# pyxploiter/HandMvNet

Hardware: AMD Instinct MI355X
Metric: samples/sec (BxV frames) eval_fps.py, 8-view 256x256; 21-kpt L2 vs reference (higher is better)
Workload: dtype f32; 1 GPU; BASELINE configs[2]: B=32/GPU x V=8 x 256x256, resnet50_paper backbone, d=524, cross_attn x5, GCN decoder; global_batch=32, views=8, frame=256, parallelism=sample-shard x1

## Files before the change

handmvnet_amd/csrc/conv_stream.hip:

```cpp
#include <cstdio>
#include <cstdlib>
#include <type_traits>
#include <utility>

#include "kernels.h"

namespace hmv {

typedef float sf32x16 __attribute__((ext_vector_type(16)));
typedef float sf32x4 __attribute__((ext_vector_type(4)));
typedef _Float16 sf16x8 __attribute__((ext_vector_type(8)));

#define HMV_SGLDS16(gptr, lptr)                                                                             \
    __builtin_amdgcn_global_load_lds((const __attribute__((address_space(1))) void *)(gptr),                \
                                     (__attribute__((address_space(3))) void *)(lptr), 16, 0, 0)

template <int N>
__device__ __forceinline__ void wait_vm() {
    static_assert(N >= 0 && N < 64, "vmcnt is a 6-bit field");
    asm volatile("s_waitcnt vmcnt(%0)" ::"n"(N) : "memory");
}
template <typename F, int... I>
__device__ __forceinline__ void static_for_impl(F &&f, std::integer_sequence<int, I...>) {
    (f(std::integral_constant<int, I>{}), ...);
}
template <int N, typename F>
__device__ __forceinline__ void static_for(F &&f) {
    static_for_impl(static_cast<F &&>(f), std::make_integer_sequence<int, N>{});
}

constexpr int sched_r(int RB, int RS, int j) { return RS ? RS : (j == 0 ? RB : 0); }
constexpr int sched_ops(int NP, int PA, int RB, int RS, int OS, int slot) { return slot < NP ? PA + sched_r(RB, RS, slot) : OS; }
constexpr int sched_after_piece(int NP, int D, int PA, int RB, int RS, int OS, int j) {
    const int T0 = 8, g = T0 * NP + j - D, tq = g / NP, jq = g - tq * NP;
    int n = sched_r(RB, RS, jq);
    for (int s = tq * (NP + 1) + jq + 1; s < T0 * (NP + 1) + j; ++s) n += sched_ops(NP, PA, RB, RS, OS, s % (NP + 1));
    return n;
}
constexpr int sched_after_residual(int NP, int PA, int RB, int RS, int OS) {
    const int T0 = 8, last = RS ? NP - 1 : 0;
    int n = 0;
    for (int s = (T0 - 1) * (NP + 1) + last + 1; s < T0 * (NP + 1) + NP; ++s) n += sched_ops(NP, PA, RB, RS, OS, s % (NP + 1));
    return n;
}
static_assert(sched_after_piece(4, 3, 1, 8, 0, 8, 0) == 10 && sched_after_piece(4, 3, 1, 8, 0, 8, 1) == 18 && sched_after_piece(4, 3, 1, 8, 0, 8, 2) == 18 &&
              sched_after_piece(4, 3, 1, 8, 0, 8, 3) == 10 && sched_after_residual(4, 1, 8, 0, 8) == 23, "the step-0 schedule of four pieces, counted by hand");
static_assert(sched_after_piece(4, 3, 1, 8, 2, 8, 0) == 2 + 3 + 3 + 8 && sched_after_residual(4, 1, 8, 2, 8) == 8 + 4 * 3, "the spread K = 256 schedule");

template <int TM, int TN, int MW, int NW, int NP, int NSLOT, bool HAS_RES, bool SPREAD = false, bool DUAL = false, int N2 = 0>
__global__ __launch_bounds__(64 * MW *NW, (MW * NW) / 4) void conv_stream_f16(const ConvParams p) {
    constexpr int NWV = MW * NW, NT = 64 * NWV;
    constexpr int BM = 32 * TM * MW, BN = 32 * TN * NW;
    constexpr int D = NSLOT - 1;
    constexpr int PA = BM * 8 / NT;
    constexpr int NB2 = N2 / 32;
    constexpr int TM2 = N2 ? (BM / 32) * NB2 / NWV : 0;
    constexpr int K2Q = BN / 16;
    static_assert(N2 == 0 || (N2 % 32 == 0 && TN == 2 && TM2 >= 1 && NWV % NB2 == 0 && (BM / 32) == (NWV / NB2) * TM2),
                  "chain: a wave's 64 output channels are one pixel piece of the second reduction; whole blocks per wave");
    constexpr int RB = HAS_RES ? TM * TN * 2 : 0, OS = TM * TN * 2 + 2 * TM2;
    constexpr int RS = (SPREAD && HAS_RES) ? RB / NP : 0;
    static_assert(!SPREAD || RB % NP == 0, "spread schedule: whole residual DMAs per step");
    constexpr int ZW = TM * TN * 2 * 1024;
    constexpr int NFAKE = (D + NP - 1) / NP;
    static_assert(NT == 512 && BM % 64 == 0 && PA >= 1, "eight waves; whole DMA passes per piece");
    static_assert((NSLOT & (NSLOT - 1)) == 0 && NSLOT >= 2, "a power of two");
    extern __shared__ __attribute__((aligned(16))) char ssm[];
    _Float16 *sA = reinterpret_cast<_Float16 *>(ssm);
    char *zones = ssm + NSLOT * BM * 128;

    const int tid = threadIdx.x, lane = tid & 63;
    const int wave = __builtin_amdgcn_readfirstlane(tid >> 6);
    const int l31 = lane & 31, kh = lane >> 5;
    const int mw = wave / NW, nw = wave - mw * NW;
    const int zi = N2 ? nw * MW + mw : wave;
    static_assert(N2 == 0 || !HAS_RES || ZW == TM * 32 * 128, "chain: a landing zone is the wave's region of the tile image");

    const int nsl = p.ntiles;
    const int loc = (int)blockIdx.x >> 3, per_xcd = 32 / nsl;
    const int slice = loc % nsl, stream = ((int)blockIdx.x & 7) * per_xcd + loc / nsl, nstreams = 8 * per_xcd;
    const int ntl = p.mtiles > stream ? (p.mtiles - stream + nstreams - 1) / nstreams : 0;
    if (ntl == 0) return;
    const int n0 = slice * BN + nw * TN * 32;

    const _Float16 *zero16 = reinterpret_cast<const _Float16 *>(p.zero);
    _Float16 *trash = reinterpret_cast<_Float16 *>(const_cast<float *>(p.zero) + 64 + 4 * lane);
    const _Float16 *Ain = reinterpret_cast<const _Float16 *>(p.in);
    const _Float16 *Rin = reinterpret_cast<const _Float16 *>(p.res);
    _Float16 *Out = reinterpret_cast<_Float16 *>(p.out);

    const int wl31 = (l31 & 0x13) | ((l31 & 4) << 1) | ((l31 & 8) >> 1);
    sf16x8 wreg[TN][NP * 4];
    {
        const _Float16 *wb = reinterpret_cast<const _Float16 *>(p.wgt) + (size_t)(n0 + wl31) * p.ldw + 8 * kh;
#pragma unroll
        for (int b = 0; b < TN; ++b)
#pragma unroll
            for (int Q = 0; Q < NP * 4; ++Q) wreg[b][Q] = *reinterpret_cast<const sf16x8 *>(wb + (size_t)(32 * b) * p.ldw + 16 * Q);
    }
    const int ob2 = N2 ? wave % (N2 ? NB2 : 1) : 0, pg2 = N2 ? wave / (N2 ? NB2 : 1) : 0;
    sf16x8 w2reg[N2 ? K2Q : 1];
    if constexpr (N2 > 0) {
        const _Float16 *wb2 = reinterpret_cast<const _Float16 *>(p.nx_wgt) + (size_t)(32 * ob2 + wl31) * p.nx_ldw + 8 * kh;
#pragma unroll
        for (int Q = 0; Q < K2Q; ++Q) w2reg[Q] = *reinterpret_cast<const sf16x8 *>(wb2 + 16 * Q);
    }
    asm volatile("s_waitcnt vmcnt(0)" ::: "memory");

    const int arow = tid >> 3, kqs = (tid & 7) ^ ((tid >> 4) & 7);
    const int fsw = (l31 >> 1) & 7;

    size_t off2[DUAL ? PA : 1] = {};
    auto issue_A = [&](int G) {
        const int tt = G >= 0 ? G / NP : -1, jj = G >= 0 ? G - tt * NP : 0, slot = G & (NSLOT - 1);
        const int mt = stream + tt * nstreams;
#pragma unroll
        for (int i = 0; i < PA; ++i) {
            const int m = mt * BM + i * 64 + arow;
            const bool ok = tt >= 0 && tt < ntl && m < p.M;
            const _Float16 *src = zero16;
            if constexpr (DUAL) {
                if (jj * 64 == p.ksplit) {
                    const int hw = p.Ho * p.Wo, n = m / hw, rem = m - n * hw, ho = rem / p.Wo, wo = rem - ho * p.Wo;
                    off2[i] = ((size_t)(n * p.H2 + ho * p.stride2) * p.W2 + wo * p.stride2) * p.lda2 + 8 * kqs;
                }
                if (ok && jj * 64 >= p.ksplit) {
                    src = reinterpret_cast<const _Float16 *>(p.in2) + off2[i] + (jj * 64 - p.ksplit);
                } else if (ok) {
                    src = Ain + (size_t)m * p.lda + jj * 64 + 8 * kqs;
                }
            } else if (ok) {
                src = Ain + (size_t)m * p.lda + jj * 64 + 8 * kqs;
            }
            asm volatile("" : "+v"(src));
            HMV_SGLDS16(src, sA + ((slot * BM + i * 64 + wave * 8) * 64));
        }
    };
    auto issue_R = [&](int tt, auto first_c, auto count_c) {
        if constexpr (HAS_RES) {
            constexpr int first = decltype(first_c)::value, count = decltype(count_c)::value;
            const int mt = stream + tt * nstreams;
            char *z = zones + ((tt & 1) * NWV + zi) * ZW;
#pragma unroll
            for (int idx = first; idx < first + count; ++idx) {
                const int a = idx / (2 * TN), b = (idx / 2) % TN, j = idx & 1;
                const int m = mt * BM + (mw * TM + a) * 32 + l31;
                const bool ok = tt >= 0 && tt < ntl && m < p.M;
                const _Float16 *src = ok ? Rin + (size_t)m * p.ldr + n0 + 32 * b + 16 * j + 8 * kh : zero16;
                asm volatile("" : "+v"(src));
                HMV_SGLDS16(src, z + idx * 1024);
            }
        }
    };
    using I0 = std::integral_constant<int, 0>;
    using IRB = std::integral_constant<int, RB>;
    using IRS = std::integral_constant<int, RS>;

#pragma unroll
    for (int ft = -NFAKE; ft < 0; ++ft) {
        static_for<NP>([&](auto jc) {
            constexpr int j = decltype(jc)::value;
            issue_A(ft * NP + j + D);
            if constexpr (RS > 0) issue_R(ft + 1, std::integral_constant<int, j * RS>{}, IRS{});
            else if constexpr (j == 0) issue_R(ft + 1, I0{}, IRB{});
        });
#pragma unroll
        for (int i = 0; i < OS; ++i)
            asm volatile("global_store_dwordx4 %0, %1, off\n\ts_nop 1" ::"v"(trash), "v"(sf32x4{0.f, 0.f, 0.f, 0.f}) : "memory");
    }

    const float lo = (p.act == ACT_RELU) ? 0.f : -INFINITY;
    const __attribute__((address_space(4))) float *bp0 =
        (const __attribute__((address_space(4))) float *)(p.bias + __builtin_amdgcn_readfirstlane(n0));
    sf32x16 acc[TM][TN];

    for (int tt = 0; tt < ntl; ++tt) {
        int bz;
        asm volatile("s_mov_b32 %0, 0" : "=s"(bz));
        const __attribute__((address_space(4))) float *bp = bp0 + bz;
#pragma unroll
        for (int b = 0; b < TN; ++b)
#pragma unroll
            for (int e = 0; e < 16; ++e) {
                const int c = 32 * b + 16 * (e >> 3) + (e & 7);
                const float v0 = bp[c], v1 = bp[c + 8];
                const float v = kh ? v1 : v0;
#pragma unroll
                for (int a = 0; a < TM; ++a) acc[a][b][e] = v;
            }
        static_for<NP>([&](auto jc) {
            constexpr int j = decltype(jc)::value;
            wait_vm<sched_after_piece(NP, D, PA, RB, RS, OS, j)>();
            asm volatile("s_waitcnt lgkmcnt(0)\n\ts_barrier" ::: "memory");
            issue_A(tt * NP + j + D);
            if constexpr (RS > 0) issue_R(tt + 1, std::integral_constant<int, j * RS>{}, IRS{});
            else if constexpr (j == 0) issue_R(tt + 1, I0{}, IRB{});
            const _Float16 *pa = sA + ((((tt * NP + j) & (NSLOT - 1)) * BM + mw * TM * 32 + l31) * 64);
#pragma unroll
            for (int q = 0; q < 4; ++q) {
                sf16x8 px[TM];
#pragma unroll
                for (int a = 0; a < TM; ++a) px[a] = *reinterpret_cast<const sf16x8 *>(pa + a * 32 * 64 + (((2 * q + kh) ^ fsw) * 8));
#pragma unroll
                for (int a = 0; a < TM; ++a)
#pragma unroll
                    for (int b = 0; b < TN; ++b)
                        acc[a][b] = __builtin_amdgcn_mfma_f32_32x32x16_f16(wreg[b][4 * j + q], px[a], acc[a][b], 0, 0, 0);
            }
        });
        if constexpr (HAS_RES) wait_vm<sched_after_residual(NP, PA, RB, RS, OS)>();
        const int mt = stream + tt * nstreams;
        const char *z = zones + ((tt & 1) * NWV + zi) * ZW + lane * 16;
        if constexpr (N2 > 0) {
            char *yt = HAS_RES ? zones + (tt & 1) * NWV * ZW : zones;
            sf16x8 rr[TM][TN][2], hv[TM][TN][2];
            if constexpr (HAS_RES) {
#pragma unroll
                for (int a = 0; a < TM; ++a)
#pragma unroll
                    for (int b = 0; b < TN; ++b)
#pragma unroll
                        for (int j = 0; j < 2; ++j) rr[a][b][j] = *reinterpret_cast<const sf16x8 *>(z + ((a * TN + b) * 2 + j) * 1024);
            }
#pragma unroll
            for (int a = 0; a < TM; ++a) {
                const int m = mt * BM + (mw * TM + a) * 32 + l31;
                _Float16 *orow = Out + (size_t)m * p.ldc + n0 + 8 * kh;
#pragma unroll
                for (int b = 0; b < TN; ++b)
#pragma unroll
                    for (int j = 0; j < 2; ++j) {
                        sf16x8 r = {0, 0, 0, 0, 0, 0, 0, 0};
                        if constexpr (HAS_RES) r = rr[a][b][j];
#pragma unroll
                        for (int u = 0; u < 8; ++u) hv[a][b][j][u] = (_Float16)fmaxf(acc[a][b][8 * j + u] * p.acc_scale + (float)r[u], lo);
                        _Float16 *dst = m < p.M ? orow + 32 * b + 16 * j : trash;
                        asm volatile("global_store_dwordx4 %0, %1, off\n\ts_nop 1" ::"v"(dst), "v"(hv[a][b][j]) : "memory");
                        if constexpr (!HAS_RES) {
                            const unsigned ya = (unsigned)(size_t)(__attribute__((address_space(3))) char *)yt +
                                                (unsigned)((nw * BM + (mw * TM + a) * 32 + l31) * 128 + (((4 * b + 2 * j + kh) ^ fsw) * 16));
                            asm volatile("ds_write_b128 %0, %1" ::"v"(ya), "v"(hv[a][b][j]) : "memory");
                        }
                    }
            }
            if constexpr (HAS_RES) {
#pragma unroll
            for (int a = 0; a < TM; ++a)
#pragma unroll
                for (int b = 0; b < TN; ++b)
#pragma unroll
                    for (int j = 0; j < 2; ++j) {
                        const unsigned ya = (unsigned)(size_t)(__attribute__((address_space(3))) char *)yt +
                                            (unsigned)((nw * BM + (mw * TM + a) * 32 + l31) * 128 + (((4 * b + 2 * j + kh) ^ fsw) * 16));
                        asm volatile("ds_write_b128 %0, %1" ::"v"(ya), "v"(hv[a][b][j]) : "memory");
                    }
            }
            asm volatile("s_waitcnt lgkmcnt(0)\n\ts_barrier" ::: "memory");
            const __attribute__((address_space(4))) float *bq =
                (const __attribute__((address_space(4))) float *)(p.nx_bias + __builtin_amdgcn_readfirstlane(32 * ob2)) + bz;
            sf32x16 acc2[TM2];
#pragma unroll
            for (int e = 0; e < 16; ++e) {
                const int c = 16 * (e >> 3) + (e & 7);
                const float v0 = bq[c], v1 = bq[c + 8];
                const float v = kh ? v1 : v0;
#pragma unroll
                for (int a = 0; a < TM2; ++a) acc2[a][e] = v;
            }
            const unsigned yr = (unsigned)(size_t)(__attribute__((address_space(3))) char *)yt + (unsigned)((pg2 * TM2 * 32 + l31) * 128);
            constexpr int G = 4 / TM2, NG = K2Q / G;
            static_assert(K2Q % G == 0 && G * TM2 == 4, "four fragment reads per group");
            sf16x8 px[2][G][TM2];
#define HMV_CHAIN_READ_GROUP(g)                                                                                                     \
    _Pragma("unroll") for (int i = 0; i < G; ++i) _Pragma("unroll") for (int a = 0; a < TM2; ++a) {                                \
        const int Q = (g) * G + i;                                                                                                  \
        const unsigned ad = yr + (unsigned)(((Q >> 2) * BM + a * 32) * 128) + (unsigned)((((2 * (Q & 3) + kh) ^ fsw)) * 16);        \
        asm volatile("ds_read_b128 %0, %1" : "=v"(px[(g) & 1][i][a]) : "v"(ad) : "memory");                                         \
    }
            HMV_CHAIN_READ_GROUP(0)
#pragma unroll
            for (int g = 0; g < NG; ++g) {
                sf16x8(&pg)[G][TM2] = px[g & 1];
                if (g + 1 < NG) {
                    HMV_CHAIN_READ_GROUP(g + 1)
                    if constexpr (TM2 == 1) asm volatile("s_waitcnt lgkmcnt(4)" : "+v"(pg[0][0]), "+v"(pg[1][0]), "+v"(pg[2][0]), "+v"(pg[3][0]) :: "memory");
                    else asm volatile("s_waitcnt lgkmcnt(4)" : "+v"(pg[0][0]), "+v"(pg[0][1]), "+v"(pg[1][0]), "+v"(pg[1][1]) :: "memory");
                } else {
                    if constexpr (TM2 == 1) asm volatile("s_waitcnt lgkmcnt(0)" : "+v"(pg[0][0]), "+v"(pg[1][0]), "+v"(pg[2][0]), "+v"(pg[3][0]) :: "memory");
                    else asm volatile("s_waitcnt lgkmcnt(0)" : "+v"(pg[0][0]), "+v"(pg[0][1]), "+v"(pg[1][0]), "+v"(pg[1][1]) :: "memory");
                }
#pragma unroll
                for (int i = 0; i < G; ++i)
#pragma unroll
                    for (int a = 0; a < TM2; ++a) acc2[a] = __builtin_amdgcn_mfma_f32_32x32x16_f16(w2reg[g * G + i], pg[i][a], acc2[a], 0, 0, 0);
            }
#undef HMV_CHAIN_READ_GROUP
            const float lo2 = (p.nx_act == ACT_RELU) ? 0.f : -INFINITY;
            _Float16 *Out2 = reinterpret_cast<_Float16 *>(p.nx_out);
#pragma unroll
            for (int a = 0; a < TM2; ++a) {
                const int m = mt * BM + (pg2 * TM2 + a) * 32 + l31;
                _Float16 *orow = Out2 + (size_t)m * p.nx_ldc + 32 * ob2 + 8 * kh;
#pragma unroll
                for (int j = 0; j < 2; ++j) {
                    const sf16x8 r = {0, 0, 0, 0, 0, 0, 0, 0};
                    sf16x8 h2;
#pragma unroll
                    for (int u = 0; u < 8; ++u) h2[u] = (_Float16)fmaxf(acc2[a][8 * j + u] * p.acc_scale + (float)r[u], lo2);
                    _Float16 *dst = m < p.M ? orow + 16 * j : trash;
                    asm volatile("global_store_dwordx4 %0, %1, off\n\ts_nop 1" ::"v"(dst), "v"(h2) : "memory");
                }
            }
        } else {
#pragma unroll
        for (int a = 0; a < TM; ++a) {
            const int m = mt * BM + (mw * TM + a) * 32 + l31;
            _Float16 *orow = Out + (size_t)m * p.ldc + n0 + 8 * kh;
#pragma unroll
            for (int b = 0; b < TN; ++b)
#pragma unroll
                for (int j = 0; j < 2; ++j) {
                    sf16x8 r = {0, 0, 0, 0, 0, 0, 0, 0};
                    if constexpr (HAS_RES) r = *reinterpret_cast<const sf16x8 *>(z + ((a * TN + b) * 2 + j) * 1024);
                    sf16x8 hv;
#pragma unroll
                    for (int u = 0; u < 8; ++u) hv[u] = (_Float16)fmaxf(acc[a][b][8 * j + u] * p.acc_scale + (float)r[u], lo);
                    _Float16 *dst = m < p.M ? orow + 32 * b + 16 * j : trash;
                    asm volatile("global_store_dwordx4 %0, %1, off\n\ts_nop 1" ::"v"(dst), "v"(hv) : "memory");
                }
        }
        }
    }
    asm volatile("s_waitcnt vmcnt(0) lgkmcnt(0)" ::: "memory");
}

template <int TM, int TN, int MW, int NW, int NP, int NSLOT, bool HAS_RES, bool DUAL = false, bool HALF = false>
__global__ __launch_bounds__(64 * MW *NW, 2) void conv_stream_f32(const ConvParams p) {
    constexpr int NWV = MW * NW, NT = 64 * NWV;
    constexpr int BM = 32 * TM * MW, BN = 32 * TN * NW;
    constexpr int D = NSLOT - 1;
    constexpr int PA = BM * 8 / NT;
    constexpr int RB = HAS_RES ? TM * TN * 4 : 0, OS = TM * TN * 4, RS = 0;
    constexpr int ZW = TM * TN * 4 * 1024;
    constexpr int NFAKE = (D + NP - 1) / NP;
    constexpr int RPP = NT / 8;
    static_assert((NT == 512 || (HALF && NT == 256)) && BM % RPP == 0 && PA >= 1 && (!HALF || (HAS_RES && !DUAL)), "whole DMA passes per piece");
    static_assert((NSLOT & (NSLOT - 1)) == 0 && NSLOT >= 2, "a power of two");
    extern __shared__ __attribute__((aligned(16))) char ssm[];
    float *sA = reinterpret_cast<float *>(ssm);
    char *zones = ssm + NSLOT * BM * 128;

    const int tid = threadIdx.x, lane = tid & 63;
    const int wave = __builtin_amdgcn_readfirstlane(tid >> 6);
    const int l31 = lane & 31, kh = lane >> 5;
    const int mw = wave / NW, nw = wave - mw * NW;
    const int nsl = p.ntiles;
    const int loc = (int)blockIdx.x >> 3, per_xcd = ((int)gridDim.x >> 3) / nsl;
    const int slice = loc % nsl, stream = ((int)blockIdx.x & 7) * per_xcd + loc / nsl, nstreams = 8 * per_xcd;
    const int ntl = p.mtiles > stream ? (p.mtiles - stream + nstreams - 1) / nstreams : 0;
    if (ntl == 0) return;
    const int n0 = slice * BN + nw * TN * 32;

    const float *zero32 = p.zero;
    float *trash = const_cast<float *>(p.zero) + 64 + 4 * lane;
    const float *Ain = reinterpret_cast<const float *>(p.in);
    const float *Rin = reinterpret_cast<const float *>(p.res);
    float *Out = reinterpret_cast<float *>(p.out);

    sf32x4 wreg[TN][NP * 4], bias[TN][4];
    {
        const float *wb = reinterpret_cast<const float *>(p.wgt) + (size_t)(n0 + l31) * p.ldw + 4 * kh;
#pragma unroll
        for (int b = 0; b < TN; ++b) {
#pragma unroll
            for (int Q = 0; Q < NP * 4; ++Q) wreg[b][Q] = *reinterpret_cast<const sf32x4 *>(wb + (size_t)(32 * b) * p.ldw + 8 * Q);
#pragma unroll
            for (int g = 0; g < 4; ++g) bias[b][g] = *reinterpret_cast<const sf32x4 *>(p.bias + n0 + 32 * b + 8 * g + 4 * kh);
        }
    }
    asm volatile("s_waitcnt vmcnt(0)" ::: "memory");

    const int arow = tid >> 3, kqs = (tid & 7) ^ ((tid >> 4) & 7);
    const int fsw = (l31 >> 1) & 7;
    auto issue_A = [&](int G) {
        const int tt = G >= 0 ? G / NP : -1, jj = G >= 0 ? G - tt * NP : 0, slot = G & (NSLOT - 1);
        const int mt = stream + tt * nstreams;
#pragma unroll
        for (int i = 0; i < PA; ++i) {
            const int m = mt * BM + i * RPP + arow;
            const bool ok = tt >= 0 && tt < ntl && m < p.M;
            const float *src = zero32;
            if constexpr (DUAL) {
                if (ok && jj * 32 >= p.ksplit) {
                    const int hw = p.Ho * p.Wo, n = m / hw, rem = m - n * hw, ho = rem / p.Wo, wo = rem - ho * p.Wo;
                    src = reinterpret_cast<const float *>(p.in2) + ((size_t)(n * p.H2 + ho * p.stride2) * p.W2 + wo * p.stride2) * p.lda2 +
                          (jj * 32 - p.ksplit) + 4 * kqs;
                } else if (ok) {
                    src = Ain + (size_t)m * p.lda + jj * 32 + 4 * kqs;
                }
            } else if (ok) {
                src = Ain + (size_t)m * p.lda + jj * 32 + 4 * kqs;
            }
            asm volatile("" : "+v"(src));
            HMV_SGLDS16(src, sA + ((slot * BM + i * RPP + wave * 8) * 32));
        }
    };
    auto issue_R = [&](int tt) {
        if constexpr (HAS_RES) {
            const int mt = stream + tt * nstreams;
            char *z = zones + ((HALF ? 0 : (tt & 1)) * NWV + wave) * ZW;
#pragma unroll
            for (int idx = 0; idx < RB; ++idx) {
                const int a = idx / (4 * TN), b = (idx / 4) % TN, g = idx & 3;
                const int m = mt * BM + (mw * TM + a) * 32 + l31;
                const bool ok = tt >= 0 && tt < ntl && m < p.M;
                const float *src = ok ? Rin + (size_t)m * p.ldr + n0 + 32 * b + 8 * g + 4 * kh : zero32;
                asm volatile("" : "+v"(src));
                HMV_SGLDS16(src, z + idx * 1024);
            }
        }
    };
#pragma unroll
    for (int ft = -NFAKE; ft < 0; ++ft) {
        static_for<NP>([&](auto jc) {
            constexpr int j = decltype(jc)::value;
            issue_A(ft * NP + j + D);
            if constexpr (j == 0) issue_R(HALF ? ft : ft + 1);
        });
#pragma unroll
        for (int i = 0; i < OS; ++i)
            asm volatile("global_store_dwordx4 %0, %1, off\n\ts_nop 1" ::"v"(trash), "v"(sf32x4{0.f, 0.f, 0.f, 0.f}) : "memory");
    }

    const float lo = (p.act == ACT_RELU) ? 0.f : -INFINITY;
    sf32x16 acc[TM][TN];
    for (int tt = 0; tt < ntl; ++tt) {
#pragma unroll
        for (int a = 0; a < TM; ++a)
#pragma unroll
            for (int b = 0; b < TN; ++b)
#pragma unroll
                for (int e = 0; e < 16; ++e) acc[a][b][e] = 0.f;
        static_for<NP>([&](auto jc) {
            constexpr int j = decltype(jc)::value;
            wait_vm<sched_after_piece(NP, D, PA, RB, RS, OS, j)>();
            asm volatile("s_waitcnt lgkmcnt(0)\n\ts_barrier" ::: "memory");
            issue_A(tt * NP + j + D);
            if constexpr (j == 0) issue_R(HALF ? tt : tt + 1);
            const float *pa = sA + ((((tt * NP + j) & (NSLOT - 1)) * BM + mw * TM * 32 + l31) * 32);
#pragma unroll
            for (int q = 0; q < 4; ++q) {
                sf32x4 px[TM];
#pragma unroll
                for (int a = 0; a < TM; ++a) px[a] = *reinterpret_cast<const sf32x4 *>(pa + a * 32 * 32 + (((2 * q + kh) ^ fsw) * 4));
#pragma unroll
                for (int e = 0; e < 4; ++e)
#pragma unroll
                    for (int a = 0; a < TM; ++a)
#pragma unroll
                        for (int b = 0; b < TN; ++b)
                            acc[a][b] = __builtin_amdgcn_mfma_f32_32x32x2f32(wreg[b][4 * j + q][e], px[a][e], acc[a][b], 0, 0, 0);
            }
        });
        if constexpr (HAS_RES) wait_vm<HALF ? (NP - 1) * PA : sched_after_residual(NP, PA, RB, RS, OS)>();
        const int mt = stream + tt * nstreams;
        const char *z = zones + ((HALF ? 0 : (tt & 1)) * NWV + wave) * ZW + lane * 16;
#pragma unroll
        for (int a = 0; a < TM; ++a) {
            const int m = mt * BM + (mw * TM + a) * 32 + l31;
            float *orow = Out + (size_t)m * p.ldc + n0 + 4 * kh;
#pragma unroll
            for (int b = 0; b < TN; ++b)
#pragma unroll
                for (int g = 0; g < 4; ++g) {
                    sf32x4 r = {0.f, 0.f, 0.f, 0.f};
                    if constexpr (HAS_RES) r = *reinterpret_cast<const sf32x4 *>(z + ((a * TN + b) * 4 + g) * 1024);
                    sf32x4 t;
#pragma unroll
                    for (int u = 0; u < 4; ++u) t[u] = fmaxf((acc[a][b][4 * g + u] + bias[b][g][u]) + r[u], lo);
                    float *dst = m < p.M ? orow + 32 * b + 8 * g : trash;
                    asm volatile("global_store_dwordx4 %0, %1, off\n\ts_nop 1" ::"v"(dst), "v"(t) : "memory");
                }
        }
    }
    asm volatile("s_waitcnt vmcnt(0) lgkmcnt(0)" ::: "memory");
}

template <int TM, int TN, int MW, int NW, int NP, int NSLOT, bool HAS_RES, bool SPREAD = false, bool DUAL = false, int N2 = 0>
static hipError_t launch_stream_one(ConvParams p, hipStream_t s) {
    constexpr int BM = 32 * TM * MW, BN = 32 * TN * NW, NWV = MW * NW;
    constexpr size_t lds = (size_t)NSLOT * BM * 128 + (HAS_RES ? (size_t)2 * NWV * TM * TN * 2 * 1024 : (N2 ? (size_t)BM * BN * 2 : 0));
    static_assert(lds <= 160 * 1024, "LDS budget");
    auto kern = conv_stream_f16<TM, TN, MW, NW, NP, NSLOT, HAS_RES, SPREAD, DUAL, N2>;
    if (N2 && (p.Cout != BN || p.nx_cout != N2 || !p.nx_wgt || !p.nx_bias || !p.nx_out)) return hipErrorInvalidValue;
    static DeviceOnce once;
    if (const hipError_t e = once.run([&](int) { return set_max_lds(lds, kern); }); e != hipSuccess) return e;
    p.mtiles = (p.M + BM - 1) / BM;
    p.ntiles = p.Cout / BN;
    hipLaunchKernelGGL(kern, dim3(256), dim3(64 * NWV), lds, s, p);
    return hipGetLastError();
}

static int stream_bn(const ConvParams &p, int *bm = nullptr) {
    int bn = 0, m = 0;
    if (p.in2) {
        if (!p.res && p.Kpad == 128 && p.ksplit == 64 && p.Cout == 256) { bn = 256; m = 128; }
        else if (!p.res && p.Kpad == 384 && p.ksplit == 128 && p.Cout == 512) { bn = 256; m = 64; }
    } else if (p.res) {
        if (p.Kpad == 256 || p.Kpad == 128) { bn = 512; m = 64; }
        else if (p.Kpad == 64) { bn = 256; m = 128; }
    } else {
        if (p.Kpad == 256 && p.Cout == 64) { bn = 64; m = 256; }
        else if (p.Kpad == 512 && p.Cout == 128) { bn = 128; m = 128; }
        else if (p.Kpad == 256 && p.Cout == 128) { bn = 128; m = 128; }
        else if (p.Kpad == 64 && p.Cout == 64) { bn = 64; m = 256; }
    }
    if (bm) *bm = m;
    return bn;
}

static int stream32_shape(const ConvParams &p) {
    if (p.in_f16 || p.out_f16) return 0;
    if (p.in2) return (!p.res && p.Kpad == 128 && p.ksplit == 64 && p.Cout == 256 && p.lda == p.ksplit && p.lda2 % 4 == 0) ? 3 : 0;
    if (p.res) return (!p.res_f16 && (p.Kpad == 64 || p.Kpad == 128 || p.Kpad == 256) && p.Cout % 256 == 0 && 32 % (p.Cout / 256) == 0) ? 1 : 0;
    return (p.Kpad == 256 && p.Cout == 64) ? 2 : ((p.Kpad == 64 && p.Cout == 64) ? 4 : 0);
}
static bool stream32_rule(const ConvParams &p) {
    static const bool no256 = HMV_DEV_ENV("HMV_NO_STREAM32_K256") != nullptr;
    return p.res ? (p.Kpad <= 128 || (!no256 && p.Cout % 128 == 0 && 64 % (p.Cout / 128) == 0)) : true;
}

bool conv_stream_supported(const ConvParams &p, const ConvRoute &route) {
    static const int min_env = HMV_DEV_INT("HMV_STREAM_MIN_TILES", 4);
    if (route.stream == ROUTE_NEVER) return false;
    const bool force = route.stream == ROUTE_FORCE;
    const int min_tiles = force ? 0 : min_env;
    if (stream32_shape(p)) {
        static const bool off32 = HMV_DEV_ENV("HMV_NO_STREAM32") != nullptr;
        if (off32 && !force) return false;
        if (p.R != 1 || p.S != 1 || p.stride != 1 || p.pad_h || p.pad_w || p.up || p.ksl > 1 || p.phases > 1) return false;
        if (p.cwrap || p.x3_plane || p.res_split || p.out_split || p.acc_shift || p.rd_cout || p.scatter || p.rg_out || p.fill) return false;
        if (p.act != ACT_NONE && p.act != ACT_RELU) return false;
        if ((!p.in2 && p.Cin != p.Kpad) || p.K != p.Kpad) return false;
        if ((p.lda ? p.lda : p.Cin) % 4 || (p.ldw ? p.ldw : p.Kpad) % 4 || p.ldc % 4 || (p.res && p.ldr % 4)) return false;
        if (force) return true;
        const int bm32 = (p.res || p.in2) ? 64 : 128, streams32 = p.res ? 256 / (p.Cout / 256) : 256;
        return stream32_rule(p) && (long long)(p.M + bm32 - 1) / bm32 >= (long long)min_tiles * streams32;
    }
    int bm = 0;
    const int bn = stream_bn(p, &bm);
    if (!bn || !p.in_f16 || !p.out_f16 || (p.res && !p.res_f16)) return false;
    if (p.R != 1 || p.S != 1 || p.stride != 1 || p.pad_h || p.pad_w || p.up || p.ksl > 1 || p.phases > 1) return false;
    if (p.in2 && ((p.lda2 & 7) || (p.ksplit & 63) || p.lda != p.ksplit)) return false;
    if (p.cwrap || p.x3_plane || p.res_split || p.out_split || p.acc_shift || p.rd_cout || p.scatter || p.rg_out || p.fill) return false;
    if (p.act != ACT_NONE && p.act != ACT_RELU) return false;
    if ((!p.in2 && p.Cin != p.Kpad) || p.K != p.Kpad || p.Cout % bn != 0 || 32 % (p.Cout / bn) != 0) return false;
    if ((p.lda ? p.lda : p.Cin) % 8 || (p.ldw ? p.ldw : p.Kpad) % 8 || p.ldc % 8 || (p.res && p.ldr % 8)) return false;
    const int streams = 256 / (p.Cout / bn);
    return (long long)(p.M + bm - 1) / bm >= (long long)min_tiles * streams;
}

bool conv_stream_chain_ok(const ConvParams &q, int nx_cout, const ConvRoute &route) {
    static const bool off = HMV_DEV_ENV("HMV_NO_CHAIN") != nullptr;
    if (off || (nx_cout != 64 && nx_cout != 128)) return false;
    ConvParams p = q;
    p.nx_wgt = nullptr;
    if (!p.lda) p.lda = p.Cin;
    if (!p.ldw) p.ldw = p.Kpad;
    if (!p.in_f16 || !p.out_f16 || p.acc_shift || p.Cout != 256 || (p.ldc & 7)) return false;
    if (!(p.in2 ? (!p.res && p.Kpad == 128 && p.ksplit == 64 && nx_cout == 64) : (p.res && p.Kpad == 64))) return false;
    return conv_stream_supported(p, route);
}

template <int TM, int TN, int MW, int NW, int NP, int NSLOT, bool HAS_RES, bool DUAL = false, bool HALF = false>
static hipError_t launch_stream32(ConvParams p, hipStream_t s) {
    constexpr int BM = 32 * TM * MW, BN = 32 * TN * NW;
    constexpr size_t lds = (size_t)NSLOT * BM * 128 + (HAS_RES ? (size_t)(HALF ? 1 : 2) * MW * NW * TM * TN * 4 * 1024 : 0);
    static_assert(lds * (HALF ? 2 : 1) <= 160 * 1024, "LDS budget");
    auto kern = conv_stream_f32<TM, TN, MW, NW, NP, NSLOT, HAS_RES, DUAL, HALF>;
    static DeviceOnce once;
    if (const hipError_t e = once.run([&](int) { return set_max_lds(lds, kern); }); e != hipSuccess) return e;
    p.mtiles = (p.M + BM - 1) / BM;
    p.ntiles = p.Cout / BN;
    hipLaunchKernelGGL(kern, dim3(HALF ? 512 : 256), dim3(64 * MW * NW), lds, s, p);
    return hipGetLastError();
}

hipError_t launch_conv_stream(const ConvParams &p, hipStream_t s, const char **name) {
    if (const int k32 = stream32_shape(p)) {
        if (k32 == 2) { if (name) *name = "conv_stream_f32<128x64,k256>"; return launch_stream32<1, 1, 4, 2, 8, 8, false>(p, s); }
        if (k32 == 4) { if (name) *name = "conv_stream_f32<128x64,k64>"; return launch_stream32<1, 1, 4, 2, 2, 8, false>(p, s); }
        if (k32 == 3) { if (name) *name = "conv_stream_f32<64x256,k128,dual>"; return launch_stream32<2, 1, 1, 8, 4, 8, false, true>(p, s); }
        if (p.Kpad == 256 && p.Cout % 128 == 0 && 64 % (p.Cout / 128) == 0) {
            if (name) *name = "conv_stream_f32<64x128,k256,res>";
            return launch_stream32<2, 1, 1, 4, 8, 4, true, false, true>(p, s);
        }
        if (p.Kpad == 256) { if (name) *name = "conv_stream_f32<64x256,k256,res>"; return launch_stream32<2, 1, 1, 8, 8, 4, true>(p, s); }
        if (p.Kpad == 128) { if (name) *name = "conv_stream_f32<64x256,k128,res>"; return launch_stream32<2, 1, 1, 8, 4, 4, true>(p, s); }
        if (name) *name = "conv_stream_f32<64x256,k64,res>";
        return launch_stream32<2, 1, 1, 8, 2, 4, true>(p, s);
    }
    if (p.nx_wgt) {
        if (p.nx_ldw < p.Cout || (p.nx_ldw & 7) || (p.nx_ldc & 7) || (p.nx_act != ACT_NONE && p.nx_act != ACT_RELU) || p.acc_shift) return hipErrorInvalidValue;
        if (p.in2 && p.Kpad == 128 && p.nx_cout == 64) {
            if (name) *name = "conv_stream_f16<128x256,k128,dual,+1x1:64>";
            return launch_stream_one<2, 2, 2, 4, 2, 4, false, false, true, 64>(p, s);
        }
        if (p.res && p.Kpad == 64 && p.nx_cout == 64) {
            if (name) *name = "conv_stream_f16<128x256,k64,res,+1x1:64>";
            return launch_stream_one<2, 2, 2, 4, 1, 2, true, false, false, 64>(p, s);
        }
        if (p.res && p.Kpad == 64 && p.nx_cout == 128) {
            if (name) *name = "conv_stream_f16<128x256,k64,res,+1x1:128>";
            return launch_stream_one<2, 2, 2, 4, 1, 2, true, false, false, 128>(p, s);
        }
        return hipErrorInvalidValue;
    }
    if (p.in2) {
        if (p.Kpad == 128) {
            if (name) *name = "conv_stream_f16<128x256,k128,dual>";
            return launch_stream_one<2, 2, 2, 4, 2, 8, false, false, true>(p, s);
        }
        if (name) *name = "conv_stream_f16<64x256,k384,dual>";
        return launch_stream_one<2, 1, 1, 8, 6, 8, false, false, true>(p, s);
    }
    if (!p.res) {
        if (p.Kpad == 256 && p.Cout == 64) {
            if (name) *name = "conv_stream_f16<256x64,k256>";
            return launch_stream_one<1, 2, 8, 1, 4, 4, false>(p, s);
        }
        if (p.Kpad == 64 && p.Cout == 64) {
            if (name) *name = "conv_stream_f16<256x64,k64>";
            return launch_stream_one<1, 2, 8, 1, 1, 4, false>(p, s);
        }
        if (p.Kpad == 512) {
            if (name) *name = "conv_stream_f16<128x128,k512>";
            return launch_stream_one<2, 1, 2, 4, 8, 8, false>(p, s);
        }
        if (name) *name = "conv_stream_f16<128x128,k256>";
        return launch_stream_one<1, 2, 4, 2, 4, 8, false>(p, s);
    }
    if (p.Kpad == 256) {
        if (name) *name = "conv_stream_f16<64x512,k256,res>";
        return launch_stream_one<2, 2, 1, 8, 4, 4, true, true>(p, s);
    }
    if (p.Kpad == 128) {
        if (name) *name = "conv_stream_f16<64x512,k128,res>";
        return launch_stream_one<2, 2, 1, 8, 2, 4, true>(p, s);
    }
    if (p.Kpad == 64) {
        if (name) *name = "conv_stream_f16<128x256,k64,res>";
        return launch_stream_one<2, 2, 2, 4, 1, 2, true>(p, s);
    }
    return hipErrorInvalidValue;
}

}
```

Measured before the change: 6179 frames/s.

## Overlap previous tile's epilogue stores with current tile MFMAs in f32 stream conv

Adds an OVL path to the f32 streaming 1x1 conv kernel. It double-buffers the accumulators and interleaves the previous tile's bias/residual/ReLU epilogue stores and the next tile's residual DMA between the current tile's MFMA groups, with explicit vmcnt wait counts derived from the schedule. The bias moves into an LDS table. The path is enabled for the k128 dual and k128 residual shapes, and the latter's ring grows from 4 to 8 slots. The aim is to hide the separate epilogue and store phase behind compute, at the cost of doubled accumulator registers and a fragile hand-counted wait schedule.

New measurement: 6193 frames/s, median of 6. Within noise of the previous version (+0.2%).

```diff
diff --git a/handmvnet_amd/csrc/conv_stream.hip b/handmvnet_amd/csrc/conv_stream.hip
--- a/handmvnet_amd/csrc/conv_stream.hip
+++ b/handmvnet_amd/csrc/conv_stream.hip
@@ -334,7 +334,13 @@
     asm volatile("s_waitcnt vmcnt(0) lgkmcnt(0)" ::: "memory");
 }
 
-template <int TM, int TN, int MW, int NW, int NP, int NSLOT, bool HAS_RES, bool DUAL = false, bool HALF = false>
+constexpr int sched32_ops(int PA, int EG, int R) { return PA + EG * (1 + R); }
+constexpr int sched32_after_piece(int D, int PA, int EG, int R) { return EG * (1 + R) + (D - 2) * sched32_ops(PA, EG, R); }
+constexpr int sched32_after_residual(int NP, int PA, int EG) { return NP * sched32_ops(PA, EG, 1) - 1; }
+static_assert(sched32_after_piece(7, 1, 2, 1) == 4 + 5 * 5 && sched32_after_residual(4, 1, 2) == 3 * 5 + 4, "64x256,k128,res: slot = pixel DMA, 2 x (store, residual DMA); seven pieces ahead");
+static_assert(sched32_after_piece(7, 1, 2, 0) == 2 + 5 * 3, "64x256,k128,dual: slot = pixel DMA, 2 stores");
+
+template <int TM, int TN, int MW, int NW, int NP, int NSLOT, bool HAS_RES, bool DUAL = false, bool HALF = false, bool OVL = false>
 __global__ __launch_bounds__(64 * MW *NW, 2) void conv_stream_f32(const ConvParams p) {
     constexpr int NWV = MW * NW, NT = 64 * NWV;
     constexpr int BM = 32 * TM * MW, BN = 32 * TN * NW;
@@ -374,9 +380,18 @@
         for (int b = 0; b < TN; ++b) {
 #pragma unroll
             for (int Q = 0; Q < NP * 4; ++Q) wreg[b][Q] = *reinterpret_cast<const sf32x4 *>(wb + (size_t)(32 * b) * p.ldw + 8 * Q);
-#pragma unroll
-            for (int g = 0; g < 4; ++g) bias[b][g] = *reinterpret_cast<const sf32x4 *>(p.bias + n0 + 32 * b + 8 * g + 4 * kh);
-        }
+            if constexpr (!OVL) {
+#pragma unroll
+                for (int g = 0; g < 4; ++g) bias[b][g] = *reinterpret_cast<const sf32x4 *>(p.bias + n0 + 32 * b + 8 * g + 4 * kh);
+            }
+        }
+    }
+    float *btab = reinterpret_cast<float *>(zones + (HAS_RES ? NWV * ZW : 0)) + wave * (TN * 32);
+    if constexpr (OVL) {
+#pragma unroll
+        for (int b = 0; b < TN; ++b)
+            if (kh == 0) btab[32 * b + l31] = p.bias[n0 + 32 * b + l31];
+        asm volatile("s_waitcnt lgkmcnt(0)" ::: "memory");
     }
     asm volatile("s_waitcnt vmcnt(0)" ::: "memory");
 
@@ -420,6 +435,104 @@
             }
         }
     };
+    if constexpr (OVL) {
+        constexpr int NG = TM * TN * 4, EG = NG / NP, QS = 4 / EG;
+        static_assert(NG % NP == 0 && EG >= 1 && EG <= 4 && 4 % EG == 0 && D >= 2, "whole epilogue rounds per step, at most one per MFMA group");
+        constexpr int WP = sched32_after_piece(D, PA, EG, HAS_RES ? 1 : 0), WR = HAS_RES ? sched32_after_residual(NP, PA, EG) : 0;
+        const float lo = (p.act == ACT_RELU) ? 0.f : -INFINITY;
+        [[maybe_unused]] const unsigned zaddr = (unsigned)(size_t)(__attribute__((address_space(3))) char *)(zones + wave * ZW + lane * 16);
+        sf32x16 acc[2][TM][TN];
+#pragma unroll
+        for (int s = 0; s < 2; ++s)
+#pragma unroll
+            for (int a = 0; a < TM; ++a)
+#pragma unroll
+                for (int b = 0; b < TN; ++b)
+#pragma unroll
+                    for (int e = 0; e < 16; ++e) acc[s][a][b][e] = 0.f;
+        auto round_read = [&](auto idx_c) {
+            sf32x4 r = {0.f, 0.f, 0.f, 0.f};
+            if constexpr (HAS_RES) {
+                wait_vm<WR>();
+                asm volatile("ds_read_b128 %0, %1 offset:%2" : "=v"(r) : "v"(zaddr), "n"(decltype(idx_c)::value * 1024) : "memory");
+            }
+            return r;
+        };
+        auto round_store = [&](auto s_c, auto idx_c, auto dma_c, sf32x4 r, int tp, int tn) {
+            constexpr int S = decltype(s_c)::value, idx = decltype(idx_c)::value;
+            constexpr int a = idx / (4 * TN), b = (idx / 4) % TN, g = idx & 3;
+            if constexpr (HAS_RES) asm volatile("s_waitcnt lgkmcnt(0)" : "+v"(r) : : "memory");
+            const sf32x4 bv = *reinterpret_cast<const sf32x4 *>(btab + 32 * b + 8 * g + 4 * kh);
+            sf32x4 t;
+#pragma unroll
+            for (int u = 0; u < 4; ++u) {
+                t[u] = fmaxf((acc[S][a][b][4 * g + u] + bv[u]) + r[u], lo);
+                acc[S][a][b][4 * g + u] = 0.f;
+            }
+            const int m = (stream + tp * nstreams) * BM + (mw * TM + a) * 32 + l31;
+            float *dst = (tp >= 0 && m < p.M) ? Out + (size_t)m * p.ldc + n0 + 4 * kh + 32 * b + 8 * g : trash;
+            asm volatile("global_store_dwordx4 %0, %1, off\n\ts_nop 1" ::"v"(dst), "v"(t) : "memory");
+            if constexpr (HAS_RES && decltype(dma_c)::value) {
+                const int mn = (stream + tn * nstreams) * BM + (mw * TM + a) * 32 + l31;
+                const float *src = mn < p.M ? Rin + (size_t)mn * p.ldr + n0 + 32 * b + 8 * g + 4 * kh : zero32;
+                asm volatile("" : "+v"(src));
+                HMV_SGLDS16(src, zones + wave * ZW + idx * 1024);
+            }
+        };
+        sf32x4 px0[TM];
+        auto read_px = [&](int G, auto q_c, sf32x4 (&px)[TM]) {
+            const float *pa = sA + (((G & (NSLOT - 1)) * BM + mw * TM * 32 + l31) * 32);
+#pragma unroll
+            for (int a = 0; a < TM; ++a) px[a] = *reinterpret_cast<const sf32x4 *>(pa + a * 32 * 32 + (((2 * decltype(q_c)::value + kh) ^ fsw) * 4));
+        };
+        auto tile = [&](auto s_c, int tt) {
+            constexpr int S = decltype(s_c)::value;
+            static_for<NP>([&](auto jc) {
+                constexpr int j = decltype(jc)::value;
+                wait_vm<WP>();
+                asm volatile("s_waitcnt lgkmcnt(0)\n\ts_barrier" ::: "memory");
+                issue_A(tt * NP + j + D);
+                sf32x4 px[2][TM];
+#pragma unroll
+                for (int a = 0; a < TM; ++a) px[0][a] = px0[a];
+                static_for<4>([&](auto qc) {
+                    constexpr int q = decltype(qc)::value;
+                    constexpr int idx = j * EG + q / QS;
+                    if constexpr (q < 3) read_px(tt * NP + j, std::integral_constant<int, q + 1>{}, px[(q + 1) & 1]);
+                    sf32x4 r = {0.f, 0.f, 0.f, 0.f};
+                    if constexpr (q % QS == 0) r = round_read(std::integral_constant<int, idx>{});
+#pragma unroll
+                    for (int e = 0; e < 4; ++e)
+#pragma unroll
+                        for (int a = 0; a < TM; ++a)
+#pragma unroll
+                            for (int b = 0; b < TN; ++b)
+                                acc[S][a][b] = __builtin_amdgcn_mfma_f32_32x32x2f32(wreg[b][4 * j + q][e], px[q & 1][a][e], acc[S][a][b], 0, 0, 0);
+                    if constexpr (q % QS == 0)
+                        round_store(std::integral_constant<int, 1 - S>{}, std::integral_constant<int, idx>{}, std::true_type{}, r, tt - 1, tt);
+                });
+                read_px(tt * NP + j + 1, std::integral_constant<int, 0>{}, px0);
+            });
+        };
+        auto drain = [&](auto s_c, int tp) {
+            static_for<NG>([&](auto ic) { round_store(s_c, ic, std::false_type{}, round_read(ic), tp, 0); });
+        };
+#pragma unroll
+        for (int g = 0; g < D; ++g) issue_A(g);
+        wait_vm<(D - 1) * PA>();
+        asm volatile("s_waitcnt lgkmcnt(0)\n\ts_barrier" ::: "memory");
+        read_px(0, std::integral_constant<int, 0>{}, px0);
+        for (int tt = 0;;) {
+            tile(std::integral_constant<int, 0>{}, tt);
+            if (++tt == ntl) break;
+            tile(std::integral_constant<int, 1>{}, tt);
+            if (++tt == ntl) break;
+        }
+        if ((ntl - 1) & 1) drain(std::integral_constant<int, 1>{}, ntl - 1);
+        else drain(std::integral_constant<int, 0>{}, ntl - 1);
+        asm volatile("s_waitcnt vmcnt(0) lgkmcnt(0)" ::: "memory");
+        return;
+    }
 #pragma unroll
     for (int ft = -NFAKE; ft < 0; ++ft) {
         static_for<NP>([&](auto jc) {
@@ -572,12 +685,13 @@
     return conv_stream_supported(p, route);
 }
 
-template <int TM, int TN, int MW, int NW, int NP, int NSLOT, bool HAS_RES, bool DUAL = false, bool HALF = false>
+template <int TM, int TN, int MW, int NW, int NP, int NSLOT, bool HAS_RES, bool DUAL = false, bool HALF = false, bool OVL = false>
 static hipError_t launch_stream32(ConvParams p, hipStream_t s) {
     constexpr int BM = 32 * TM * MW, BN = 32 * TN * NW;
-    constexpr size_t lds = (size_t)NSLOT * BM * 128 + (HAS_RES ? (size_t)(HALF ? 1 : 2) * MW * NW * TM * TN * 4 * 1024 : 0);
+    constexpr size_t lds = (size_t)NSLOT * BM * 128 + (HAS_RES ? (size_t)((HALF || OVL) ? 1 : 2) * MW * NW * TM * TN * 4 * 1024 : 0) +
+                           (OVL ? (size_t)MW * NW * TN * 128 : 0);
     static_assert(lds * (HALF ? 2 : 1) <= 160 * 1024, "LDS budget");
-    auto kern = conv_stream_f32<TM, TN, MW, NW, NP, NSLOT, HAS_RES, DUAL, HALF>;
+    auto kern = conv_stream_f32<TM, TN, MW, NW, NP, NSLOT, HAS_RES, DUAL, HALF, OVL>;
     static DeviceOnce once;
     if (const hipError_t e = once.run([&](int) { return set_max_lds(lds, kern); }); e != hipSuccess) return e;
     p.mtiles = (p.M + BM - 1) / BM;
@@ -590,13 +704,13 @@
     if (const int k32 = stream32_shape(p)) {
         if (k32 == 2) { if (name) *name = "conv_stream_f32<128x64,k256>"; return launch_stream32<1, 1, 4, 2, 8, 8, false>(p, s); }
         if (k32 == 4) { if (name) *name = "conv_stream_f32<128x64,k64>"; return launch_stream32<1, 1, 4, 2, 2, 8, false>(p, s); }
-        if (k32 == 3) { if (name) *name = "conv_stream_f32<64x256,k128,dual>"; return launch_stream32<2, 1, 1, 8, 4, 8, false, true>(p, s); }
+        if (k32 == 3) { if (name) *name = "conv_stream_f32<64x256,k128,dual>"; return launch_stream32<2, 1, 1, 8, 4, 8, false, true, false, true>(p, s); }
         if (p.Kpad == 256 && p.Cout % 128 == 0 && 64 % (p.Cout / 128) == 0) {
             if (name) *name = "conv_stream_f32<64x128,k256,res>";
             return launch_stream32<2, 1, 1, 4, 8, 4, true, false, true>(p, s);
         }
         if (p.Kpad == 256) { if (name) *name = "conv_stream_f32<64x256,k256,res>"; return launch_stream32<2, 1, 1, 8, 8, 4, true>(p, s); }
-        if (p.Kpad == 128) { if (name) *name = "conv_stream_f32<64x256,k128,res>"; return launch_stream32<2, 1, 1, 8, 4, 4, true>(p, s); }
+        if (p.Kpad == 128) { if (name) *name = "conv_stream_f32<64x256,k128,res>"; return launch_stream32<2, 1, 1, 8, 4, 8, true, false, false, true>(p, s); }
         if (name) *name = "conv_stream_f32<64x256,k64,res>";
         return launch_stream32<2, 1, 1, 8, 2, 4, true>(p, s);
     }
```
